# facebook/zstd

Hardware: NVIDIA H100
Metric: compress GB/s (input) at level 1 (higher is better)
Workload: dtype u8

## Files before the change

### zstd_b200/csrc/zb_match.cu

```cuda
#include "zb_device.cuh"
#include "zb_kernels.h"
#include "zb_merge.cuh"

template <bool DICT>
__device__ __forceinline__ u32 zb_count_fwd(const ZbSeg& sg, u32 a, u32 offset, u32 be, u32 lane)
{
    u32 fwd = 0;
    while (true) {
        u32 const pa = a + fwd + 8u * lane;
        u32 m;
        if (pa + 8u <= be) {
            u64 const x = zb_seg_ld64x<DICT>(sg, pa) ^ zb_seg_ld64x<DICT>(sg, pa - offset);
            m = x ? (u32)((__ffsll((long long)x) - 1) >> 3) : 8u;
        } else {
            m = 0;
            while (pa + m < be && zb_seg_byte<DICT>(sg, pa + m) == zb_seg_byte<DICT>(sg, pa + m - offset)) m++;
        }
        u32 const inc = __ballot_sync(ZB_FULL, m != 8u);
        if (inc == 0) { fwd += 256u; continue; }
        int const f = __ffs((int)inc) - 1;
        fwd += 8u * (u32)f + __shfl_sync(ZB_FULL, m, f);
        return fwd;
    }
}
// ... 443 lines not shown
        bool const act = (p < se) && (p + 9u <= be);
        u32 const pp = act ? p : ip;
        u32 dL = act ? zb_dist_at(dLp, fLp, pp - bs) : 0u;
        u32 dS = act ? zb_dist_at(dSp, fSp, pp - bs) : 0u;
        u32 dL1 = act ? zb_dist_at(dLp, fLp, pp + 1u - bs) : 0u;
        if (dL > pp) dL = 0u;
        if (dS > pp) dS = 0u;
        if (dL1 > pp + 1u) dL1 = 0u;
        u64 const w = zb_seg_ld64x<DICT>(sg, pp);
        u32 const cur = (u32)w, cur1 = (u32)(w >> 8);
        bool const v2 = act && rep1 != 0u && (p + 1u >= rep1);
        u32 const r2 = (u32)zb_seg_ld64x<DICT>(sg, v2 ? pp + 1u - rep1 : pp);
        u32 r3 = ~cur;
        bool const v3 = (lane == 0u) && (ip == anchor) && (rep2 != 0u);
        if (ip == anchor && rep2 != 0u) r3 = (u32)zb_seg_ld64x<DICT>(sg, v3 ? pp - rep2 : pp);
        u32 hit = (v3 && r3 == cur) ? 3u : ((v2 && r2 == cur1) ? 2u : (dL ? 1u : (dS ? 4u : 0u)));
        u32 tent = __ballot_sync(ZB_FULL, hit != 0u);
        u32 ms = 0, offset = 0, mlen = 0, wtype = 0;
        bool found = false;
        while (tent) {
            int const winner = __ffs((int)tent) - 1;
            u32 const probe = __shfl_sync(ZB_FULL, p, winner);
            wtype = __shfl_sync(ZB_FULL, hit, winner);
            u32 const wL = __shfl_sync(ZB_FULL, dL, winner), wS = __shfl_sync(ZB_FULL, dS, winner), wL1 = __shfl_sync(ZB_FULL, dL1, winner);
            if (wtype == 3u) { ms = probe; offset = rep2; mlen = 4u + zb_count_fwd<DICT>(sg, probe + 4u, rep2, be, lane); found = true; break; }
            if (wtype == 2u) { ms = probe + 1u; offset = rep1; mlen = 4u + zb_count_fwd<DICT>(sg, probe + 5u, rep1, be, lane); found = true; break; }
            if (wtype == 1u) {
                u32 const f0 = zb_count_fwd<DICT>(sg, probe, wL, be, lane);
                if (f0 >= 8u) {
                    u32 const back = zb_back_coop<DICT>(sg, probe, wL, anchor, lane);
                    ms = probe - back; offset = wL; mlen = back + f0; found = true; break;
                }
                if (lane == (u32)winner) hit = dS ? 4u : 0u;
                if (wS == 0u) { tent &= ~(1u << winner); }
                continue;
            }
            {   u32 const f0 = zb_count_fwd<DICT>(sg, probe, wS, be, lane);
                if (f0 < 4u) { tent &= ~(1u << winner); if (lane == (u32)winner) hit = 0u; continue; }
                u32 mp = probe, mo = wS, ml = f0;
                if (wL1) {
                    u32 const f1 = zb_count_fwd<DICT>(sg, probe + 1u, wL1, be, lane);
                    if (f1 >= 8u && f1 > ml) { mp = probe + 1u; mo = wL1; ml = f1; }
                }
                u32 const back = zb_back_coop<DICT>(sg, mp, mo, anchor, lane);
                ms = mp - back; offset = mo; mlen = back + ml; wtype = 1u; found = true; break;
            }
        }
        if (!found) { ip += 32u * step; continue; }
        if (wtype == 3u) { u32 const t = rep2; rep2 = rep1; rep1 = t; }
        else if (wtype == 1u) { rep2 = rep1; rep1 = offset; }
        if (lane == 0) myseq[nbSeq] = zb_pack_raw(offset, mlen, ms - bs);
        nbSeq++;
        ip = ms + mlen; anchor = ip; searchStart = ip;
    }
    if (lane == 0) { ZbSegMeta z; z.nbSeq = nbSeq; z.pad[0] = z.pad[1] = z.pad[2] = 0; segmeta[(size_t)b * segs + k] = z; }
}

struct ZbRepHist { u32 r1, r2, r3; };
__device__ __forceinline__ u32 zb_rep_code(ZbRepHist& h, u32 off, u32 ll)
{
    u32 code;
    if (ll > 0u) {
        if (off == h.r1) return 1u;
        if (off == h.r2) { code = 2u; h.r2 = h.r1; h.r1 = off; return code; }
        if (off == h.r3) { code = 3u; h.r3 = h.r2; h.r2 = h.r1; h.r1 = off; return code; }
    } else {
        if (off == h.r2) { code = 1u; h.r2 = h.r1; h.r1 = off; return code; }
        if (off == h.r3) { code = 2u; h.r3 = h.r2; h.r2 = h.r1; h.r1 = off; return code; }
        if (h.r1 > 1u && off == h.r1 - 1u) { code = 3u; h.r3 = h.r2; h.r2 = h.r1; h.r1 = off; return code; }
    }
    h.r3 = h.r2; h.r2 = h.r1; h.r1 = off;
    return off + 3u;
}

#ifndef MERGE_MIN_CTAS
#define MERGE_MIN_CTAS 6
#endif
#define SEG_SLOTS (ZB_PARSE_SEG / 4u)

__device__ __forceinline__ u32 zb_block_excl(bool flag, u32* wsum, u32* total)
{
    u32 const lane = threadIdx.x & 31u, warp = threadIdx.x >> 5;
    u32 const bal = __ballot_sync(ZB_FULL, flag);
    if (lane == 0u) wsum[warp] = __popc(bal);
    __syncthreads();
    u32 before = __popc(bal & ((1u << lane) - 1u)), t = 0;
    for (u32 w = 0; w < MERGE_THREADS / 32u; w++) { if (w < warp) before += wsum[w]; t += wsum[w]; }
    __syncthreads();
    *total = t;
    return before;
}

__device__ __forceinline__ void zb_ldm_clip(u32 ms, u32 me, const u64* L, u32 nL, u32* ms2, u32* me2, u32* next, bool* kept)
{
    u32 lo = 0, hi = nL;
    while (lo < hi) { u32 const mid = (lo + hi) >> 1; if (ZB_LDM_START(L[mid]) <= ms) lo = mid + 1u; else hi = mid; }
    bool clipped = false;
    if (lo > 0u && ZB_LDM_START(L[lo - 1u]) + ZB_LDM_LEN(L[lo - 1u]) > ms) { ms = ZB_LDM_START(L[lo - 1u]) + ZB_LDM_LEN(L[lo - 1u]); clipped = true; }
    if (lo < nL && ZB_LDM_START(L[lo]) < me) { me = ZB_LDM_START(L[lo]); clipped = true; }
    *ms2 = ms; *me2 = me; *next = lo;
    *kept = me > ms && (!clipped || me - ms >= 4u);
}
__device__ u32 zb_ldm_overlay(const u64* __restrict__ P, u32 nP, const u64* __restrict__ L, u32 nL, u32* __restrict__ kp, u64* __restrict__ out,
                              u32* wsum, u32* sEnd, u32& carry)
{
    u32 const tid = threadIdx.x;
    u32 base = 0;
    for (u32 i0 = 0; i0 < nP; i0 += MERGE_THREADS) {
        u32 const i = i0 + tid;
        u32 ms2, me2, nx; bool kept = false;
        if (i < nP) { u64 const r = P[i]; zb_ldm_clip(ZB_RAW_MS(r), ZB_RAW_MS(r) + ZB_RAW_MLEN(r), L, nL, &ms2, &me2, &nx, &kept); }
        u32 t;
        u32 const before = zb_block_excl(kept, wsum, &t);
        if (i < nP) kp[i] = base + before;
        base += t;
    }
    if (tid == 0) kp[nP] = base;
    __syncthreads();
    for (u32 i = tid; i < nP; i += MERGE_THREADS) {
        u64 const r = P[i];
        u32 ms2, me2, nx; bool kept;
        zb_ldm_clip(ZB_RAW_MS(r), ZB_RAW_MS(r) + ZB_RAW_MLEN(r), L, nL, &ms2, &me2, &nx, &kept);
        if (kept) out[kp[i] + nx] = zb_pack_ldm(ms2, me2 - ms2, ZB_RAW_OFF(r));
    }
    for (u32 k = tid; k < nL; k += MERGE_THREADS) {
        u32 const s = ZB_LDM_START(L[k]);
        u32 lo = 0, hi = nP;
        while (lo < hi) { u32 const mid = (lo + hi) >> 1; if (ZB_RAW_MS(P[mid]) < s) lo = mid + 1u; else hi = mid; }
        out[k + kp[lo]] = L[k];
    }
    u32 const n = base + nL;
    __syncthreads();
    if (tid == 0) carry = 0;
    for (u32 o0 = 0; o0 < n; o0 += MERGE_THREADS) {
        u32 const o = o0 + tid;
        u64 const m = o < n ? out[o] : 0ull;
        sEnd[tid] = ZB_LDM_START(m) + ZB_LDM_LEN(m);
        __syncthreads();
        u32 const prevEnd = tid ? sEnd[tid - 1u] : carry;
        if (o < n) out[o] = zb_pack_seq(ZB_LDM_OFF(m), ZB_LDM_START(m) - prevEnd, ZB_LDM_LEN(m));
        __syncthreads();
        if (tid == MERGE_THREADS - 1u) carry = sEnd[tid];
        __syncthreads();
    }
    return n;
}

template <bool LDM>
__global__ void __launch_bounds__(MERGE_THREADS, MERGE_MIN_CTAS)
zb_merge_segments_kernel(const u8* __restrict__ src, const ZbDictSlot* __restrict__ dicts, const ZbBlock* __restrict__ blocks, ZbStrides sd, const ZbSegMeta* __restrict__ segmeta,
                         u64* __restrict__ seqs, u8* __restrict__ lits, ZbBlockMeta* __restrict__ meta,
                         ZbLdmView ldm, u32* __restrict__ farScratch, u16* __restrict__ distScratch)
{
    __shared__ u32 sPos[MERGE_TILE], sLit[MERGE_TILE], sLen[MERGE_TILE], sOff[MERGE_TILE];
    __shared__ u32 wsumL[MERGE_THREADS / 32], wsumA[MERGE_THREADS / 32], wmaxU[MERGE_THREADS / 32], wmaxK[MERGE_THREADS / 32];
    __shared__ u32 sR2[MERGE_TILE], sRep[3];
    __shared__ u32 baseL, baseA, carryEnd;
    __shared__ u32 gFirst[ZB_PARSE_SEGS], gCnt[ZB_PARSE_SEGS], gBase[ZB_PARSE_SEGS], gCur[ZB_PARSE_SEGS], gPm[ZB_PARSE_SEGS], gPl[ZB_PARSE_SEGS];
    __shared__ u32 gTotal;
    u32 const b = blockIdx.x, tid = threadIdx.x, lane = tid & 31u, warp = tid >> 5;
    ZbBlock const bd = blocks[b];
    if (bd.size < 7u) return;
    u64* const myseq = seqs + (size_t)b * sd.seq;
    u8*  const mylit = lits + (size_t)b * sd.lit;
    const u8* const in = src + bd.srcOff;
    u32 const segs = (bd.size + ZB_PARSE_SEG - 1u) / ZB_PARSE_SEG;
    u32 const segStride = zb_segsPerRow(sd);
    if (warp == 0u) {
        u32 nb = 0; u64 r0 = 0, rl = 0;
        if (lane < segs) {
            nb = segmeta[(size_t)b * segStride + lane].nbSeq;
            if (nb) { r0 = myseq[(size_t)lane * SEG_SLOTS]; rl = myseq[(size_t)lane * SEG_SLOTS + nb - 1u]; }
        }
        u32 cur = 0, total = 0;
        for (u32 k = 0; k < segs; k++) {
            u32 const n = __shfl_sync(ZB_FULL, nb, (int)k);
            u64 r = __shfl_sync(ZB_FULL, r0, (int)k);
            u64 const last = __shfl_sync(ZB_FULL, rl, (int)k);
            u32 f = 0, pm = 0, pl = 0;
            while (f < n) {
                u32 const ms = ZB_RAW_MS(r), ml = ZB_RAW_MLEN(r);
                if (ms + ml <= cur || (ms < cur && ms + ml - cur < 3u)) { f++; if (f < n) r = myseq[(size_t)k * SEG_SLOTS + f]; continue; }
                if (ms < cur) { pm = cur; pl = ms + ml - cur; } else { pm = ms; pl = ml; }
                break;
            }
            if (lane == 0u) { gFirst[k] = f; gCnt[k] = n - f; gBase[k] = total; gCur[k] = cur; gPm[k] = pm; gPl[k] = pl; }
            if (f < n) { cur = (f == n - 1u) ? pm + pl : ZB_RAW_MS(last) + ZB_RAW_MLEN(last); total += n - f; }
        }
        if (lane == 0u) gTotal = total;
    }
    __syncthreads();
    u32 nbSeq;
    if constexpr (LDM) {
        u64* const P = reinterpret_cast<u64*>(farScratch + (size_t)b * sd.dist);
#pragma unroll 1
        for (u32 k = 0; k < segs; k++) {
            u32 const f = gFirst[k], cnt = gCnt[k];
            const u64* const sfrom = myseq + (size_t)k * SEG_SLOTS + f;
            for (u32 i = tid; i < cnt; i += MERGE_THREADS) {
                u64 r = sfrom[i];
                if (i == 0u) r = zb_pack_raw(ZB_RAW_OFF(r), gPl[k], gPm[k]);
                P[gBase[k] + i] = r;
            }
        }
        __syncthreads();
        nbSeq = zb_ldm_overlay(P, gTotal, ldm.match + ldm.first[b], ldm.cnt[b], reinterpret_cast<u32*>(distScratch + (size_t)b * sd.dist), myseq,
                               wsumA, sPos, carryEnd);
        __syncthreads();
    } else {
#pragma unroll 1
    for (u32 k = 0; k < segs; k++) {
        u32 const f = gFirst[k], cnt = gCnt[k];
        const u64* const sfrom = myseq + (size_t)k * SEG_SLOTS + f;
        u64* const sto = myseq + gBase[k];
        for (u32 c0 = 0; c0 < cnt; c0 += MERGE_THREADS) {
            u32 const i = c0 + tid;
            u64 r = 0; u32 ms = 0, ml = 0;
            if (i < cnt) { r = sfrom[i]; ms = ZB_RAW_MS(r); ml = ZB_RAW_MLEN(r); if (i == 0u) { ms = gPm[k]; ml = gPl[k]; } }
            u32 const myEnd = ms + ml;
            u32 prevEnd = __shfl_up_sync(ZB_FULL, myEnd, 1);
            if (lane == 31u) wsumL[warp] = myEnd;
            __syncthreads();
            if (lane == 0u) prevEnd = warp ? wsumL[warp - 1u] : (c0 ? carryEnd : gCur[k]);
            __syncthreads();
            if (i < cnt) sto[i] = zb_pack_seq(ZB_RAW_OFF(r), ms - prevEnd, ml);
            if (tid == MERGE_THREADS - 1u) carryEnd = myEnd;
            __syncthreads();
        }
    }
    nbSeq = gTotal;
    }
    u32 rep[3] = { 1u, 4u, 8u };
    if (dicts && (bd.flags & ZB_FLAG_FIRST)) { rep[0] = dicts[bd.dictSlot].codeRep[0]; rep[1] = dicts[bd.dictSlot].codeRep[1]; rep[2] = dicts[bd.dictSlot].codeRep[2]; }
    zb_merge_codes(rep[0], rep[1], rep[2], (bd.flags & ZB_FLAG_FIRST) != 0u, myseq, mylit, in, nbSeq, bd.size, meta + b,
                   sPos, sLit, sLen, sOff, sR2, sRep, wsumL, wsumA, wmaxU, wmaxK, baseL, baseA);
}

__global__ void __launch_bounds__(MERGE_THREADS)
zb_merge_small_kernel(const u8* __restrict__ src, const ZbDictSlot* __restrict__ dicts, const ZbBlock* __restrict__ blocks, u32 nbBlocks, ZbStrides sd, const ZbSegMeta* __restrict__ segmeta,
                      u64* __restrict__ seqs, u8* __restrict__ lits, ZbBlockMeta* __restrict__ meta)
{
    u32 const lane = threadIdx.x & 31u;
    u32 const b = blockIdx.x * (MERGE_THREADS / 32u) + (threadIdx.x >> 5);
    if (b >= nbBlocks) return;
    ZbBlock const bd = blocks[b];
    if (bd.size < 7u) return;
    u64* const myseq = seqs + (size_t)b * sd.seq;
    u8* const mylit = lits + (size_t)b * sd.lit;
    const u8* const in = src + bd.srcOff;
    u32 const nbSeq = segmeta[b].nbSeq;
    ZbRepHist hist; hist.r1 = 0; hist.r2 = 0; hist.r3 = 0;
    if (bd.flags & ZB_FLAG_FIRST) {
        hist.r1 = 1u; hist.r2 = 4u; hist.r3 = 8u;
        if (dicts) { hist.r1 = dicts[bd.dictSlot].codeRep[0]; hist.r2 = dicts[bd.dictSlot].codeRep[1]; hist.r3 = dicts[bd.dictSlot].codeRep[2]; }
    }
    u32 posL = 0, posA = 0;
    for (u32 t0 = 0; t0 < nbSeq; t0 += 32u) {
        u32 const i = t0 + lane;
        u64 const r = (i < nbSeq) ? myseq[i] : 0ull;
        u32 const ms = ZB_RAW_MS(r), ml = ZB_RAW_MLEN(r), off = ZB_RAW_OFF(r);
        u32 const myEnd = (i < nbSeq) ? ms + ml : 0u;
        u32 prevEnd = __shfl_up_sync(ZB_FULL, myEnd, 1);
        if (lane == 0u) prevEnd = posA;
        u32 const ll = (i < nbSeq) ? ms - prevEnd : 0u;
        u32 const adv = ll + ((i < nbSeq) ? ml : 0u);
        u32 inL = ll;
#pragma unroll
        for (u32 o = 1; o < 32u; o <<= 1) { u32 const x = __shfl_up_sync(ZB_FULL, inL, o); if (lane >= o) inL += x; }
        u32 code = 0;
        u32 const cnt = min(32u, nbSeq - t0);
        for (u32 j = 0; j < cnt; j++) {
            u32 const o = __shfl_sync(ZB_FULL, off, (int)j), l = __shfl_sync(ZB_FULL, ll, (int)j);
            u32 const c = zb_rep_code(hist, o, l);
            if (lane == j) code = c;
        }
        if (i < nbSeq) {
            const u8* const from = in + prevEnd;
            u8* const to = mylit + posL + inL - ll;
            for (u32 x = 0; x < ll; x++) to[x] = from[x];
            myseq[i] = zb_pack_seq(code, ll, ml);
        }
        posL += __shfl_sync(ZB_FULL, inL, 31);
        posA = __shfl_sync(ZB_FULL, myEnd, (int)(cnt - 1u));
        (void)adv;
    }
    u32 const lastLits = bd.size - posA;
    for (u32 x = lane; x < lastLits; x += 32u) mylit[posL + x] = in[posA + x];
    if (lane == 0) {
        ZbBlockMeta m; m.nbSeq = nbSeq; m.litSize = posL + lastLits; m.litSecSize = 0; m.bodySize = 0;
        m.type = ZB_BT_COMPRESSED; m.forceRaw = 0; m.rleByte = 0; m.pad = 0;
        meta[b] = m;
    }
}

template <int MLS, int P>
static cudaError_t zb_launch_walk_p(const u8* d_src, const ZbDictSlot* d_dicts, const ZbChunk* d_chunks, u32 nbChunks, u32 N, u32 insStep, const ZbStrides& sd,
                                    u32 slotFirstBlock, u16* d_dist, u32* d_far, u32 imageOff, bool build, cudaStream_t stream)
{
    cudaError_t const e = cudaFuncSetAttribute(zb_walk_kernel<MLS, P>, cudaFuncAttributeMaxDynamicSharedMemorySize, 226 * 1024);
    if (e != cudaSuccess) return e;
    zb_walk_kernel<MLS, P><<<nbChunks, ZB_BATCH / P, (size_t)N * 4u, stream>>>(d_src, d_dicts, d_chunks, insStep, N, sd, slotFirstBlock, d_dist, d_far, imageOff, build);
    return cudaGetLastError();
}
template <int MLS>
static cudaError_t zb_launch_walk_m(const u8* d_src, const ZbDictSlot* d_dicts, const ZbChunk* d_chunks, u32 nbChunks, u32 N, u32 insStep, const ZbStrides& sd,
                                    u32 slotFirstBlock, u16* d_dist, u32* d_far, u32 imageOff, bool build, cudaStream_t stream)
{
    size_t const smem = (size_t)N * 4u;
    if (smem <= 56u * 1024u)  return zb_launch_walk_p<MLS, WALK_P_SMALL>(d_src, d_dicts, d_chunks, nbChunks, N, insStep, sd, slotFirstBlock, d_dist, d_far, imageOff, build, stream);
    if (smem <= 113u * 1024u) return zb_launch_walk_p<MLS, WALK_P_MID>(d_src, d_dicts, d_chunks, nbChunks, N, insStep, sd, slotFirstBlock, d_dist, d_far, imageOff, build, stream);
    return zb_launch_walk_p<MLS, 1>(d_src, d_dicts, d_chunks, nbChunks, N, insStep, sd, slotFirstBlock, d_dist, d_far, imageOff, build, stream);
}
extern "C" cudaError_t zb_launch_walk(const u8* d_src, const ZbDictSlot* d_dicts, const ZbChunk* d_chunks, u32 nbChunks, u32 mls, u32 N, u32 insStep, const ZbStrides& sd,
                                      u32 slotFirstBlock, u16* d_dist, u32* d_far, u32 imageOff, bool build, cudaStream_t stream)
{
    switch (mls) {
    case 4: return zb_launch_walk_m<4>(d_src, d_dicts, d_chunks, nbChunks, N, insStep, sd, slotFirstBlock, d_dist, d_far, imageOff, build, stream);
    case 5: return zb_launch_walk_m<5>(d_src, d_dicts, d_chunks, nbChunks, N, insStep, sd, slotFirstBlock, d_dist, d_far, imageOff, build, stream);
    case 6: return zb_launch_walk_m<6>(d_src, d_dicts, d_chunks, nbChunks, N, insStep, sd, slotFirstBlock, d_dist, d_far, imageOff, build, stream);
    case 7: return zb_launch_walk_m<7>(d_src, d_dicts, d_chunks, nbChunks, N, insStep, sd, slotFirstBlock, d_dist, d_far, imageOff, build, stream);
    default: return zb_launch_walk_m<8>(d_src, d_dicts, d_chunks, nbChunks, N, insStep, sd, slotFirstBlock, d_dist, d_far, imageOff, build, stream);
    }
}

extern "C" cudaError_t zb_launch_dict_images(const ZbDictSlot* d_dicts, const ZbChunk* d_imageChunks, u32 nbImages, const ZbParams* prm, cudaStream_t stream)
{
    if (nbImages == 0) return cudaSuccess;
    ZbStrides const sd = zb_strides(ZB_BLOCK_MAX);
    cudaError_t e = zb_launch_walk(nullptr, d_dicts, d_imageChunks, nbImages, prm->mls, prm->tableN, prm->insStep, sd, 0, nullptr, nullptr, 0, true, stream);
    if (e == cudaSuccess && prm->strategy == 2)
        e = zb_launch_walk(nullptr, d_dicts, d_imageChunks, nbImages, 8, prm->tableNLong, prm->insStep, sd, 0, nullptr, nullptr, prm->tableN, true, stream);
    return e;
}

extern "C" cudaError_t zb_launch_match(const u8* d_src, const ZbDictSlot* d_dicts, bool dict, const ZbBlock* d_blocks, u32 nbBlocks,
                                       const ZbChunk* d_chunks, u32 nbChunks, u32 slotFirstBlock, const ZbParams* prm, const ZbWorkRows* rows,
                                       cudaEvent_t evMid, cudaStream_t stream, const ZbLdmView* ldm)
{
    if (nbBlocks == 0) return cudaSuccess;
    ZbStrides const sd = rows->sd;
    u16* const d_dist = rows->dist; u32* const d_far = rows->far; u16* const d_dist2 = rows->dist2; u32* const d_far2 = rows->far2;
    u64* const d_seqs = rows->seqs; ZbBlockMeta* const d_meta = rows->meta; ZbSegMeta* const d_segmeta = rows->segmeta;
    cudaError_t e;
    u32 const segs = zb_segsPerRow(sd);
    u32 const sgrid = (u32)(((u64)nbBlocks * segs + PARSE_WARPS - 1) / PARSE_WARPS);
    if (prm->strategy == 2) {
        e = zb_launch_walk(d_src, d_dicts, d_chunks, nbChunks, 8, prm->tableNLong, prm->insStep, sd, slotFirstBlock, d_dist, d_far, prm->tableN, false, stream); if (e != cudaSuccess) return e;
        e = zb_launch_walk(d_src, d_dicts, d_chunks, nbChunks, prm->mls, prm->tableN, prm->insStep, sd, slotFirstBlock, d_dist2, d_far2, 0, false, stream); if (e != cudaSuccess) return e;
        if (evMid) cudaEventRecord(evMid, stream);
        if (dict) zb_parse_dfast_kernel<true><<<sgrid, 32 * PARSE_WARPS, 0, stream>>>(d_src, d_dicts, d_blocks, nbBlocks, *prm, sd, d_dist, d_far, d_dist2, d_far2, d_seqs, d_meta, d_segmeta);
        else      zb_parse_dfast_kernel<false><<<sgrid, 32 * PARSE_WARPS, 0, stream>>>(d_src, d_dicts, d_blocks, nbBlocks, *prm, sd, d_dist, d_far, d_dist2, d_far2, d_seqs, d_meta, d_segmeta);
    } else {
        if (prm->stepSize < 2u) return cudaErrorInvalidValue;
        e = zb_launch_walk(d_src, d_dicts, d_chunks, nbChunks, prm->mls, prm->tableN, prm->insStep, sd, slotFirstBlock, d_dist, d_far, 0, false, stream); if (e != cudaSuccess) return e;
        if (evMid) cudaEventRecord(evMid, stream);
        if (dict) zb_parse_kernel<true><<<sgrid, 32 * PARSE_WARPS, 0, stream>>>(d_src, d_dicts, d_blocks, nbBlocks, *prm, sd, d_dist, d_far, d_seqs, d_meta, d_segmeta);
        else      zb_parse_kernel<false><<<sgrid, 32 * PARSE_WARPS, 0, stream>>>(d_src, d_dicts, d_blocks, nbBlocks, *prm, sd, d_dist, d_far, d_seqs, d_meta, d_segmeta);
    }
    return zb_launch_merge(d_src, d_dicts, d_blocks, nbBlocks, rows, ldm, stream);
}

extern "C" cudaError_t zb_launch_merge(const u8* d_src, const ZbDictSlot* d_dicts, const ZbBlock* d_blocks, u32 nbBlocks, const ZbWorkRows* rows,
                                       const ZbLdmView* ldm, cudaStream_t stream)
{
    if (nbBlocks == 0) return cudaSuccess;
    ZbStrides const sd = rows->sd;
    u32 const segs = zb_segsPerRow(sd);
    if (segs == 1u && sd.dist <= 8192u)
        zb_merge_small_kernel<<<(nbBlocks + MERGE_THREADS / 32u - 1u) / (MERGE_THREADS / 32u), MERGE_THREADS, 0, stream>>>(d_src, d_dicts, d_blocks, nbBlocks, sd, rows->segmeta, rows->seqs, rows->lits, rows->meta);
    else if (ldm)
        zb_merge_segments_kernel<true><<<nbBlocks, MERGE_THREADS, 0, stream>>>(d_src, d_dicts, d_blocks, sd, rows->segmeta, rows->seqs, rows->lits, rows->meta, *ldm, rows->far, rows->dist);
    else
        zb_merge_segments_kernel<false><<<nbBlocks, MERGE_THREADS, 0, stream>>>(d_src, d_dicts, d_blocks, sd, rows->segmeta, rows->seqs, rows->lits, rows->meta, ZbLdmView(), nullptr, nullptr);
    return cudaGetLastError();
}
```

### zstd_b200/csrc/zb_merge.cuh

```cuda
#ifndef ZB_MERGE_CUH
#define ZB_MERGE_CUH
#include "zb_common.h"
#include "zb_device.cuh"

#define MERGE_THREADS 256
#define MERGE_TILE 1024u
#define MERGE_PER (MERGE_TILE / MERGE_THREADS)

__device__ __forceinline__ void zb_merge_codes(u32 rep0, u32 rep1, u32 rep2, bool first, u64* __restrict__ myseq, u8* __restrict__ mylit,
                                               const u8* __restrict__ in, u32 nbSeq, u32 blockSize, ZbBlockMeta* __restrict__ metaOut,
                                               u32* sPos, u32* sLit, u32* sLen, u32* sOff, u32* sR2, u32* sRep,
                                               u32* wsumL, u32* wsumA, u32* wmaxU, u32* wmaxK, u32& baseL, u32& baseA)
{
    u32 const tid = threadIdx.x, lane = tid & 31u, warp = tid >> 5;
    if (tid == 0) {
        baseL = 0; baseA = 0;
        sRep[0] = first ? rep0 : 0u; sRep[1] = first ? rep1 : 0u; sRep[2] = first ? rep2 : 0u;
    }
    __syncthreads();
    for (u32 t0 = 0; t0 < nbSeq; t0 += MERGE_TILE) {
        u32 const n = min(MERGE_TILE, nbSeq - t0);
        u32 ll[MERGE_PER], adv[MERGE_PER], ml[MERGE_PER], off[MERGE_PER], myL = 0, myA = 0;
#pragma unroll
        for (u32 j = 0; j < MERGE_PER; j++) {
            u32 const i = tid * MERGE_PER + j;
            u64 const q = (i < n) ? myseq[t0 + i] : 0ull;
            ll[j] = ZB_SEQ_LL(q);
            ml[j] = ZB_SEQ_ML(q);
            adv[j] = ll[j] + ml[j];
            off[j] = ZB_SEQ_OFFBASE(q);
            if (i < n) sOff[i] = off[j];
            myL += ll[j]; myA += adv[j];
        }
        u32 inL = myL, inA = myA;
#pragma unroll
        for (u32 o = 1; o < 32u; o <<= 1) {
            u32 const a = __shfl_up_sync(ZB_FULL, inL, o), c = __shfl_up_sync(ZB_FULL, inA, o);
            if (lane >= o) { inL += a; inA += c; }
        }
        if (lane == 31u) { wsumL[warp] = inL; wsumA[warp] = inA; }
        u32 const R1 = sRep[0], R2 = sRep[1], R3 = sRep[2];
        __syncthreads();
        u32 offL = baseL + inL - myL, offA = baseA + inA - myA;
        for (u32 w = 0; w < warp; w++) { offL += wsumL[w]; offA += wsumA[w]; }
#pragma unroll
        for (u32 j = 0; j < MERGE_PER; j++) {
            u32 const i = tid * MERGE_PER + j;
            if (i < n) { sPos[i] = offA; sLit[i] = offL; sLen[i] = ll[j]; }
            offL += ll[j]; offA += adv[j];
        }
        u32 prevOff[MERGE_PER], r2b[MERGE_PER], r3b[MERGE_PER], bef[MERGE_PER];
        bool U[MERGE_PER], K[MERGE_PER];
        u32 run = 0;
#pragma unroll
        for (u32 j = 0; j < MERGE_PER; j++) {
            u32 const i = tid * MERGE_PER + j;
            prevOff[j] = j ? off[j - 1u] : (i == 0u ? R1 : ((i < n) ? sOff[i - 1u] : 0u));
            U[j] = ll[j] > 0u && off[j] == prevOff[j];
            bef[j] = run;
            if (i < n && !U[j]) run = i + 1u;
        }
        {   u32 inc = run;
#pragma unroll
            for (u32 o = 1; o < 32u; o <<= 1) { u32 const x = __shfl_up_sync(ZB_FULL, inc, o); if (lane >= o) inc = max(inc, x); }
            if (lane == 31u) wmaxU[warp] = inc;
            u32 ex = __shfl_up_sync(ZB_FULL, inc, 1); if (lane == 0u) ex = 0u;
            __syncthreads();
            for (u32 w = 0; w < warp; w++) ex = max(ex, wmaxU[w]);
#pragma unroll
            for (u32 j = 0; j < MERGE_PER; j++) {
                u32 const i = tid * MERGE_PER + j;
                u32 const m = max(bef[j], ex);
                r2b[j] = m == 0u ? R2 : (m == 1u ? R1 : sOff[m - 2u]);
                if (i < n) sR2[i] = r2b[j];
            }
        }
        if (tid == MERGE_THREADS - 1u) { baseL = offL; baseA = offA; }
        run = 0;
#pragma unroll
        for (u32 j = 0; j < MERGE_PER; j++) {
            u32 const i = tid * MERGE_PER + j;
            K[j] = U[j] || off[j] == r2b[j];
            bef[j] = run;
            if (i < n && !K[j]) run = i + 1u;
        }
        {   u32 inc = run;
#pragma unroll
            for (u32 o = 1; o < 32u; o <<= 1) { u32 const x = __shfl_up_sync(ZB_FULL, inc, o); if (lane >= o) inc = max(inc, x); }
            if (lane == 31u) wmaxK[warp] = inc;
            u32 ex = __shfl_up_sync(ZB_FULL, inc, 1); if (lane == 0u) ex = 0u;
            __syncthreads();
            for (u32 w = 0; w < warp; w++) ex = max(ex, wmaxK[w]);
#pragma unroll
            for (u32 j = 0; j < MERGE_PER; j++) {
                u32 const i = tid * MERGE_PER + j;
                u32 const m = max(bef[j], ex);
                r3b[j] = m == 0u ? R3 : sR2[m - 1u];
                bool const swp = !U[j] && off[j] == r2b[j];
                u32 c = off[j] + 3u;
                if (ll[j] > 0u) { if (U[j]) c = 1u; else if (swp) c = 2u; else if (off[j] == r3b[j]) c = 3u; }
                else            { if (swp) c = 1u; else if (off[j] == r3b[j]) c = 2u; else if (prevOff[j] > 1u && off[j] == prevOff[j] - 1u) c = 3u; }
                if (i < n) myseq[t0 + i] = zb_pack_seq(c, ll[j], ml[j]);
                if (i == n - 1u) { sRep[0] = off[j]; sRep[1] = U[j] ? r2b[j] : prevOff[j]; sRep[2] = K[j] ? r3b[j] : r2b[j]; }
            }
        }
        {   u32 const L0 = sLit[0], L1 = sLit[n - 1u] + sLen[n - 1u];
            for (u32 g = (L0 >> 3) + tid; (g << 3) < L1; g += MERGE_THREADS) {
                u32 const jb = g << 3;
                u32 const j0 = jb > L0 ? jb : L0, j1 = jb + 8u < L1 ? jb + 8u : L1;
                u32 sq = 0;
#pragma unroll
                for (u32 stp = MERGE_TILE / 2u; stp > 0u; stp >>= 1) {
                    u32 const c = sq + stp;
                    if (c < n && sLit[c] <= j0) sq = c;
                }
                u32 runEnd = sLit[sq] + sLen[sq];
                const u8* from = in + (sPos[sq] - sLit[sq]);
                u64 v = 0;
#pragma unroll
                for (u32 k = 0; k < 8u; k++) {
                    u32 const j = jb + k;
                    if (j >= j0 && j < j1) {
                        while (j >= runEnd) { sq++; runEnd = sLit[sq] + sLen[sq]; from = in + (sPos[sq] - sLit[sq]); }
                        v |= (u64)from[j] << (8u * k);
                    }
                }
                if (j1 - j0 == 8u) *reinterpret_cast<u64*>(mylit + jb) = v;
                else for (u32 j = j0; j < j1; j++) mylit[j] = (u8)(v >> (8u * (j - jb)));
            }
        }
        __syncthreads();
    }
    u32 const litSeq = baseL, consumed = baseA;
    u32 const lastLits = blockSize - consumed;
    for (u32 x = tid; x < lastLits; x += MERGE_THREADS) mylit[litSeq + x] = in[consumed + x];
    if (tid == 0) {
        ZbBlockMeta m; m.nbSeq = nbSeq; m.litSize = litSeq + lastLits; m.litSecSize = 0; m.bodySize = 0;
        m.type = ZB_BT_COMPRESSED; m.forceRaw = 0; m.rleByte = 0; m.pad = 0;
        *metaOut = m;
    }
}
#endif
```

### zstd_b200/csrc/zb_seqimport.cu

```cuda
#include "zb_device.cuh"
#include "zb_kernels.h"
#include "zb_merge.cuh"

#define SEQ_THREADS 256u
#define SEQ_TILE 1024u
#define SEQ_PER (SEQ_TILE / SEQ_THREADS)

__device__ __forceinline__ bool zb_isDelim(uint4 q, bool expl) { return expl && q.x == 0u && q.z == 0u; }

__device__ __forceinline__ void zb_scan2(u64& a, u32& b, u64* wa, u32* wb, u64* totA, u32* totB)
{
    u32 const lane = threadIdx.x & 31u, warp = threadIdx.x >> 5;
#pragma unroll
    for (u32 o = 1; o < 32u; o <<= 1) {
        u64 const x = __shfl_up_sync(ZB_FULL, a, o); u32 const y = __shfl_up_sync(ZB_FULL, b, o);
        if (lane >= o) { a += x; b += y; }
    }
    if (lane == 31u) { wa[warp] = a; wb[warp] = b; }
    __syncthreads();
    u64 pa = 0; u32 pb = 0;
    for (u32 w = 0; w < warp; w++) { pa += wa[w]; pb += wb[w]; }
    if (totA) { u64 ta = 0; u32 tb = 0; for (u32 w = 0; w < blockDim.x / 32u; w++) { ta += wa[w]; tb += wb[w]; } *totA = ta; *totB = tb; }
    a += pa; b += pb;
    __syncthreads();
// ... 12 lines not shown
#pragma unroll
    for (u32 k = 0; k < SEQ_PER; k++) {
        u32 const i = t0 + k * SEQ_THREADS + tid;
        sq[k * SEQ_THREADS + tid] = i < n ? seqs[i] : make_uint4(0u, 0u, 0u, 0u);
    }
    bool prevDelim = false;
    if (tid == 0 && t0 > 0) prevDelim = zb_isDelim(seqs[t0 - 1u], expl);
    __syncthreads();
    u64 len[SEQ_PER]; bool end[SEQ_PER];
    u64 a = 0; u32 c = 0;
#pragma unroll
    for (u32 k = 0; k < SEQ_PER; k++) {
        u32 const j = tid * SEQ_PER + k;
        uint4 const q = sq[j];
        bool const pd = j ? zb_isDelim(sq[j - 1u], expl) : prevDelim;
        bool const d = zb_isDelim(q, expl);
        len[k] = (u64)q.y + q.z;
        end[k] = t0 + j < n && d && (q.y > 0u || (t0 + j > 0u && !pd));
        a += len[k]; c += end[k];
    }
    u64 const myA = a; u32 const myC = c;
    if (!PLACE) {
        u64 ta; u32 tb;
        zb_scan2(a, c, wa, wb, &ta, &tb);
        if (tid == 0) { tileLen[blockIdx.x] = ta; tileEnds[blockIdx.x] = tb; }
        return;
    }
    zb_scan2(a, c, wa, wb, nullptr, nullptr);
    u64 p = tileLen[blockIdx.x] + a - myA;
    u32 k0 = tileEnds[blockIdx.x] + c - myC;
    u32 bad = ~0u;
#pragma unroll
    for (u32 k = 0; k < SEQ_PER; k++) {
        u32 const j = tid * SEQ_PER + k, i = t0 + j;
        if (i >= n) break;
        uint4 const q = sq[j];
        u64 const s = p;
        p += len[k];
        if (!zb_isDelim(q, expl)) {
            u64 const bound = p > window ? window : p + dictContent;
            if (q.x == 0u || q.z < 3u || (u64)q.x > bound || q.x > ZB_SEQ_OFF_MAX) bad = min(bad, i);
        }
        if (p > srcSize) bad = min(bad, i);
        if (expl) {
            if (end[k] && k0 < nbBlocks) { blockEnd[k0] = p; blockSeq[k0] = i; }
            k0 += end[k];
        } else if (p > s && s < srcSize) {
            for (u64 b = (s + blockMax - 1u) / blockMax; b < nbBlocks && b * blockMax < p; b++) { blockFirst[b] = i; blockFirstPos[b] = s; }
        }
    }
    if (bad != ~0u) atomicMin(errIdx, (unsigned long long)bad);
}

__global__ void __launch_bounds__(SEQ_THREADS)
zb_seq_scan_kernel(u64* __restrict__ tileLen, u32* __restrict__ tileEnds, u32 nbTiles, u64* __restrict__ ctrl)
{
    __shared__ u64 wa[SEQ_THREADS / 32u]; __shared__ u32 wb[SEQ_THREADS / 32u];
    __shared__ u64 carryA; __shared__ u32 carryB;
    if (threadIdx.x == 0) { carryA = 0; carryB = 0; }
    __syncthreads();
    for (u32 t0 = 0; t0 < nbTiles; t0 += SEQ_THREADS) {
        u32 const i = t0 + threadIdx.x;
        u64 a = i < nbTiles ? tileLen[i] : 0ull; u32 b = i < nbTiles ? tileEnds[i] : 0u;
        u64 const myA = a; u32 const myB = b;
        u64 ta; u32 tb;
        zb_scan2(a, b, wa, wb, &ta, &tb);
        if (i < nbTiles) { tileLen[i] = carryA + a - myA; tileEnds[i] = carryB + b - myB; }
        __syncthreads();
        if (threadIdx.x == 0) { carryA += ta; carryB += tb; }
        __syncthreads();
    }
    if (threadIdx.x == 0) { ctrl[0] = carryA; ctrl[1] = carryB; }
}

__global__ void zb_seq_blocks_kernel(const u64* __restrict__ blockEnd, const u32* __restrict__ blockSeq, u32 nbBlocks, u32 blockMax, u32 dictFlag,
                                     ZbBlock* __restrict__ blocks, u32* __restrict__ blockFirst, u64* __restrict__ blockFirstPos,
                                     u64* __restrict__ ctrl, unsigned long long* __restrict__ errIdx)
{
    u32 const k = blockIdx.x * blockDim.x + threadIdx.x;
    if (k >= nbBlocks) return;
    u64 const start = k ? blockEnd[k - 1u] : 0ull, e = blockEnd[k];
    if (e - start > blockMax) atomicMin(errIdx, (unsigned long long)blockSeq[k]);
    ZbBlock b; b.srcOff = start; b.size = (u32)min(e - start, (u64)blockMax); b.histLen = 0; b.frame = 0; b.dictLen = 0; b.dictSlot = 0;
    b.flags = (k == 0u ? ZB_FLAG_FIRST | dictFlag : 0u) | (k + 1u == nbBlocks ? ZB_FLAG_LAST : 0u);
    blocks[k] = b;
    blockFirst[k] = k ? blockSeq[k - 1u] + 1u : 0u;
    blockFirstPos[k] = start;
    if (k + 1u == nbBlocks) ctrl[3] = e;
}

__global__ void __launch_bounds__(MERGE_THREADS)
zb_seq_convert_kernel(const u8* __restrict__ src, const ZbBlock* __restrict__ blocks, const u32* __restrict__ blockFirst, const u64* __restrict__ blockFirstPos,
                      const uint4* __restrict__ seqsIn, u32 n, const ZbDictSlot* __restrict__ dicts, ZbStrides sd,
                      u64* __restrict__ seqs, u8* __restrict__ lits, ZbBlockMeta* __restrict__ meta)
{
    __shared__ u32 sPos[MERGE_TILE], sLit[MERGE_TILE], sLen[MERGE_TILE], sOff[MERGE_TILE];
    __shared__ u32 wsumL[MERGE_THREADS / 32], wsumA[MERGE_THREADS / 32], wmaxU[MERGE_THREADS / 32], wmaxK[MERGE_THREADS / 32];
    __shared__ u32 sR2[MERGE_TILE], sRep[3];
    __shared__ u32 baseL, baseA;
    __shared__ u64 wa[MERGE_THREADS / 32]; __shared__ u32 wb[MERGE_THREADS / 32];
    __shared__ long long carryP; __shared__ u32 carryK, carryEnd;
    u32 const b = blockIdx.x, tid = threadIdx.x, lane = tid & 31u, warp = tid >> 5;
    ZbBlock const bd = blocks[b];
    if (bd.size < 7u) {
        if (tid == 0) {
            ZbBlockMeta m; m.nbSeq = 0; m.litSize = bd.size; m.litSecSize = 0; m.bodySize = bd.size;
            m.type = ZB_BT_RAW; m.forceRaw = 1; m.rleByte = 0; m.pad = 0;
            meta[b] = m;
        }
        return;
    }
    u64* const myseq = seqs + (size_t)b * sd.seq;
    u8*  const mylit = lits + (size_t)b * sd.lit;
    const u8* const in = src + bd.srcOff;
    u32 const first = blockFirst[b];
    long long const E = bd.size;
    if (tid == 0) { carryP = first < n ? (long long)blockFirstPos[b] - (long long)bd.srcOff : E; carryK = 0; carryEnd = 0; }
    __syncthreads();
    for (u32 i0 = first; i0 < n; i0 += MERGE_THREADS) {
        u32 const i = i0 + tid;
        uint4 const q = i < n ? seqsIn[i] : make_uint4(0u, 0u, 0u, 0u);
        long long const base = carryP;
        if (base >= E) break;
        u64 a = (u64)q.y + q.z; u32 unused = 0;
        u64 const myLen = a;
        zb_scan2(a, unused, wa, wb, nullptr, nullptr);
        long long const s = base + (long long)(a - myLen), m = s + q.y, e = m + q.z;
        long long const ms = m > 0 ? m : 0, me = e < E ? e : E;
        bool const keep = i < n && s < E && me >= ms + 3;
        u32 const kb = __ballot_sync(ZB_FULL, keep);
        u32 const before = __popc(kb & ((1u << lane) - 1u));
        u32 const kEnd = keep ? (u32)me : 0u;
        u32 inc = kEnd;
#pragma unroll
        for (u32 o = 1; o < 32u; o <<= 1) { u32 const x = __shfl_up_sync(ZB_FULL, inc, o); if (lane >= o) inc = max(inc, x); }
        if (lane == 31u) { wsumL[warp] = __popc(kb); wmaxU[warp] = inc; }
        __syncthreads();
        u32 cnt = carryK, prevEnd = carryEnd;
        for (u32 w = 0; w < warp; w++) { cnt += wsumL[w]; prevEnd = max(prevEnd, wmaxU[w]); }
        u32 ex = __shfl_up_sync(ZB_FULL, inc, 1);
        if (lane > 0u) prevEnd = max(prevEnd, ex);
        if (keep) myseq[cnt + before] = zb_pack_seq(q.x, (u32)ms - prevEnd, (u32)(me - ms));
        __syncthreads();
        if (tid == MERGE_THREADS - 1u) {
            u32 tk = 0, te = carryEnd;
            for (u32 w = 0; w < MERGE_THREADS / 32u; w++) { tk += wsumL[w]; te = max(te, wmaxU[w]); }
            carryK += tk; carryEnd = te; carryP = s + (i < n ? (long long)myLen : 0ll);
            if (i + 1u >= n) carryP = E;
        }
        __syncthreads();
    }
    u32 rep[3] = { 1u, 4u, 8u };
    if (dicts && (bd.flags & ZB_FLAG_FIRST)) { rep[0] = dicts[bd.dictSlot].codeRep[0]; rep[1] = dicts[bd.dictSlot].codeRep[1]; rep[2] = dicts[bd.dictSlot].codeRep[2]; }
    zb_merge_codes(rep[0], rep[1], rep[2], (bd.flags & ZB_FLAG_FIRST) != 0u, myseq, mylit, in, carryK, bd.size, meta + b,
                   sPos, sLit, sLen, sOff, sR2, sRep, wsumL, wsumA, wmaxU, wmaxK, baseL, baseA);
}

extern "C" cudaError_t zb_launch_seq_partition(const void* d_seqs, u32 n, int expl, u64* d_tileLen, u32* d_tileEnds, u64* d_ctrl, cudaStream_t stream)
{
    if (n == 0) return cudaSuccess;
    u32 const nbTiles = (n + SEQ_TILE - 1u) / SEQ_TILE;
    zb_seq_tiles_kernel<false><<<nbTiles, SEQ_THREADS, 0, stream>>>((const uint4*)d_seqs, n, expl != 0, d_tileLen, d_tileEnds, 0, 0, 0, 0, 0,
                                                                   nullptr, nullptr, nullptr, nullptr, nullptr);
    zb_seq_scan_kernel<<<1, SEQ_THREADS, 0, stream>>>(d_tileLen, d_tileEnds, nbTiles, d_ctrl);
    return cudaGetLastError();
}

extern "C" cudaError_t zb_launch_seq_place(const void* d_seqs, u32 n, int expl, const u64* d_tileLen, const u32* d_tileEnds,
                                           u64 srcSize, u64 window, u64 dictContent, u32 blockMax, u32 nbBlocks,
                                           u64* d_blockEnd, u32* d_blockSeq, u32* d_blockFirst, u64* d_blockFirstPos, u64* d_ctrl, cudaStream_t stream)
{
    if (n == 0) return cudaSuccess;
    u32 const nbTiles = (n + SEQ_TILE - 1u) / SEQ_TILE;
    zb_seq_tiles_kernel<true><<<nbTiles, SEQ_THREADS, 0, stream>>>((const uint4*)d_seqs, n, expl != 0, (u64*)d_tileLen, (u32*)d_tileEnds,
                                                                  srcSize, window, dictContent, blockMax, nbBlocks,
                                                                  d_blockEnd, d_blockSeq, d_blockFirst, d_blockFirstPos, (unsigned long long*)(d_ctrl + 2));
    return cudaGetLastError();
}

extern "C" cudaError_t zb_launch_seq_blocks(const u64* d_blockEnd, const u32* d_blockSeq, u32 nbBlocks, u32 blockMax, u32 dictFlag,
                                            ZbBlock* d_blocks, u32* d_blockFirst, u64* d_blockFirstPos, u64* d_ctrl, cudaStream_t stream)
{
    if (nbBlocks == 0) return cudaSuccess;
    zb_seq_blocks_kernel<<<(nbBlocks + 255u) / 256u, 256, 0, stream>>>(d_blockEnd, d_blockSeq, nbBlocks, blockMax, dictFlag, d_blocks, d_blockFirst,
                                                                      d_blockFirstPos, d_ctrl, (unsigned long long*)(d_ctrl + 2));
    return cudaGetLastError();
}

extern "C" cudaError_t zb_launch_seq_convert(const u8* d_src, const ZbBlock* d_blocks, u32 nbBlocks, const u32* d_blockFirst, const u64* d_blockFirstPos,
                                             const void* d_seqs, u32 n, const ZbDictSlot* d_dicts, const ZbWorkRows* rows, cudaStream_t stream)
{
    if (nbBlocks == 0) return cudaSuccess;
    zb_seq_convert_kernel<<<nbBlocks, MERGE_THREADS, 0, stream>>>(d_src, d_blocks, d_blockFirst, d_blockFirstPos, (const uint4*)d_seqs, n, d_dicts, rows->sd,
                                                                 rows->seqs, rows->lits, rows->meta);
    return cudaGetLastError();
}
```

Baseline: 113.9.

## Parallelize segment merge across warps and gather literals with 64-bit loads

Replaces the serial warp-0 scan over parse segments with one warp per segment that finds its first surviving sequence by ballot. A single flat pass then compacts all survivors into the far scratch buffer, using binary search over segment bases and the preceding element for literal length, instead of a per-segment tiled scan with three barriers per tile. The code-merge step reads from that scratch buffer, and literal gathering now copies whole runs with unaligned 64-bit loads rather than byte by byte. This adds scratch traffic on the non-LDM path and relies on an assumption that segment count equals warps per block.

```diff
diff --git a/zstd_b200/csrc/zb_match.cu b/zstd_b200/csrc/zb_match.cu
--- a/zstd_b200/csrc/zb_match.cu
+++ b/zstd_b200/csrc/zb_match.cu
@@ -619,11 +619,13 @@
                          u64* __restrict__ seqs, u8* __restrict__ lits, ZbBlockMeta* __restrict__ meta,
                          ZbLdmView ldm, u32* __restrict__ farScratch, u16* __restrict__ distScratch)
 {
+    static_assert(ZB_PARSE_SEGS == MERGE_THREADS / 32, "step 1 reads one parse segment per warp");
     __shared__ u32 sPos[MERGE_TILE], sLit[MERGE_TILE], sLen[MERGE_TILE], sOff[MERGE_TILE];
     __shared__ u32 wsumL[MERGE_THREADS / 32], wsumA[MERGE_THREADS / 32], wmaxU[MERGE_THREADS / 32], wmaxK[MERGE_THREADS / 32];
     __shared__ u32 sR2[MERGE_TILE], sRep[3];
     __shared__ u32 baseL, baseA, carryEnd;
     __shared__ u32 gFirst[ZB_PARSE_SEGS], gCnt[ZB_PARSE_SEGS], gBase[ZB_PARSE_SEGS], gCur[ZB_PARSE_SEGS], gPm[ZB_PARSE_SEGS], gPl[ZB_PARSE_SEGS];
+    __shared__ u32 gLastMs[ZB_PARSE_SEGS], gLastEnd[ZB_PARSE_SEGS];
     __shared__ u32 gTotal;
     u32 const b = blockIdx.x, tid = threadIdx.x, lane = tid & 31u, warp = tid >> 5;
     ZbBlock const bd = blocks[b];
@@ -632,74 +634,66 @@
     u8*  const mylit = lits + (size_t)b * sd.lit;
     const u8* const in = src + bd.srcOff;
     u32 const segs = (bd.size + ZB_PARSE_SEG - 1u) / ZB_PARSE_SEG;
-    u32 const segStride = zb_segsPerRow(sd);
-    if (warp == 0u) {
-        u32 nb = 0; u64 r0 = 0, rl = 0;
-        if (lane < segs) {
-            nb = segmeta[(size_t)b * segStride + lane].nbSeq;
-            if (nb) { r0 = myseq[(size_t)lane * SEG_SLOTS]; rl = myseq[(size_t)lane * SEG_SLOTS + nb - 1u]; }
-        }
-        u32 cur = 0, total = 0;
-        for (u32 k = 0; k < segs; k++) {
-            u32 const n = __shfl_sync(ZB_FULL, nb, (int)k);
-            u64 r = __shfl_sync(ZB_FULL, r0, (int)k);
-            u64 const last = __shfl_sync(ZB_FULL, rl, (int)k);
-            u32 f = 0, pm = 0, pl = 0;
-            while (f < n) {
-                u32 const ms = ZB_RAW_MS(r), ml = ZB_RAW_MLEN(r);
-                if (ms + ml <= cur || (ms < cur && ms + ml - cur < 3u)) { f++; if (f < n) r = myseq[(size_t)k * SEG_SLOTS + f]; continue; }
-                if (ms < cur) { pm = cur; pl = ms + ml - cur; } else { pm = ms; pl = ml; }
-                break;
-            }
-            if (lane == 0u) { gFirst[k] = f; gCnt[k] = n - f; gBase[k] = total; gCur[k] = cur; gPm[k] = pm; gPl[k] = pl; }
-            if (f < n) { cur = (f == n - 1u) ? pm + pl : ZB_RAW_MS(last) + ZB_RAW_MLEN(last); total += n - f; }
-        }
-        if (lane == 0u) gTotal = total;
-    }
-    __syncthreads();
-    u32 nbSeq;
+    u32 const nb = warp < segs ? segmeta[(size_t)b * zb_segsPerRow(sd) + warp].nbSeq : 0u;
+    const u64* const seg = myseq + (size_t)warp * SEG_SLOTS;
+    u64 r = lane < nb ? seg[lane] : 0ull;
+    if (lane == 0u) {
+        u64 const last = nb ? seg[nb - 1u] : 0ull;
+        gLastMs[warp] = ZB_RAW_MS(last); gLastEnd[warp] = ZB_RAW_MS(last) + ZB_RAW_MLEN(last);
+    }
+    __syncthreads();
+    u32 cur = 0;
+#pragma unroll
+    for (u32 k = 0; k < ZB_PARSE_SEGS - 1u; k++) {
+        u32 const ms = gLastMs[k], e = gLastEnd[k];
+        if (k < warp && !(e <= cur || (ms < cur && e - cur < 3u))) cur = e;
+    }
+    u32 f = 0;
+    for (;;) {
+        u32 const ms = ZB_RAW_MS(r), e = ms + ZB_RAW_MLEN(r);
+        u32 const drop = __ballot_sync(ZB_FULL, f + lane < nb && (e <= cur || (ms < cur && e - cur < 3u)));
+        if (drop != ZB_FULL) { f += __ffs(~drop) - 1u; break; }
+        f += 32u;
+        r = f + lane < nb ? seg[f + lane] : 0ull;
+    }
+    r = __shfl_sync(ZB_FULL, r, (int)(f & 31u));
+    if (lane == 0u) {
+        u32 const ms = ZB_RAW_MS(r), ml = ZB_RAW_MLEN(r);
+        gFirst[warp] = f; gCnt[warp] = nb - f; gCur[warp] = cur;
+        gPm[warp] = ms < cur ? cur : ms; gPl[warp] = ms < cur ? ms + ml - cur : ml;
+    }
+    __syncthreads();
+    if (tid < ZB_PARSE_SEGS) {
+        u32 before = 0, total = 0;
+        for (u32 k = 0; k < ZB_PARSE_SEGS; k++) { before += k < tid ? gCnt[k] : 0u; total += gCnt[k]; }
+        gBase[tid] = before;
+        if (tid == 0u) gTotal = total;
+    }
+    __syncthreads();
+    u64* const P = reinterpret_cast<u64*>(farScratch + (size_t)b * sd.dist);
+    u32 const nbSurv = gTotal;
+    for (u32 i = tid; i < nbSurv; i += MERGE_THREADS) {
+        u32 k = 0;
+#pragma unroll
+        for (u32 st = ZB_PARSE_SEGS / 2u; st > 0u; st >>= 1) if (gBase[k + st] <= i) k += st;
+        u32 const j = i - gBase[k];
+        const u64* const from = myseq + (size_t)k * SEG_SLOTS + gFirst[k] + j;
+        u64 const q = from[0];
+        u64 const qp = (!LDM && j) ? from[-1] : 0ull;
+        u32 ms = ZB_RAW_MS(q), ml = ZB_RAW_MLEN(q), prevEnd = ZB_RAW_MS(qp) + ZB_RAW_MLEN(qp);
+        if (j == 0u) { ms = gPm[k]; ml = gPl[k]; prevEnd = gCur[k]; }
+        P[i] = LDM ? zb_pack_raw(ZB_RAW_OFF(q), ml, ms) : zb_pack_seq(ZB_RAW_OFF(q), ms - prevEnd, ml);
+    }
+    __syncthreads();
+    u32 nbSeq = nbSurv;
     if constexpr (LDM) {
-        u64* const P = reinterpret_cast<u64*>(farScratch + (size_t)b * sd.dist);
-#pragma unroll 1
-        for (u32 k = 0; k < segs; k++) {
-            u32 const f = gFirst[k], cnt = gCnt[k];
-            const u64* const sfrom = myseq + (size_t)k * SEG_SLOTS + f;
-            for (u32 i = tid; i < cnt; i += MERGE_THREADS) {
-                u64 r = sfrom[i];
-                if (i == 0u) r = zb_pack_raw(ZB_RAW_OFF(r), gPl[k], gPm[k]);
-                P[gBase[k] + i] = r;
-            }
-        }
-        __syncthreads();
-        nbSeq = zb_ldm_overlay(P, gTotal, ldm.match + ldm.first[b], ldm.cnt[b], reinterpret_cast<u32*>(distScratch + (size_t)b * sd.dist), myseq,
+        nbSeq = zb_ldm_overlay(P, nbSurv, ldm.match + ldm.first[b], ldm.cnt[b], reinterpret_cast<u32*>(distScratch + (size_t)b * sd.dist), myseq,
                                wsumA, sPos, carryEnd);
         __syncthreads();
-    } else {
-#pragma unroll 1
-    for (u32 k = 0; k < segs; k++) {
-        u32 const f = gFirst[k], cnt = gCnt[k];
-        const u64* const sfrom = myseq + (size_t)k * SEG_SLOTS + f;
-        u64* const sto = myseq + gBase[k];
-        for (u32 c0 = 0; c0 < cnt; c0 += MERGE_THREADS) {
-            u32 const i = c0 + tid;
-            u64 r = 0; u32 ms = 0, ml = 0;
-            if (i < cnt) { r = sfrom[i]; ms = ZB_RAW_MS(r); ml = ZB_RAW_MLEN(r); if (i == 0u) { ms = gPm[k]; ml = gPl[k]; } }
-            u32 const myEnd = ms + ml;
-            u32 prevEnd = __shfl_up_sync(ZB_FULL, myEnd, 1);
-            if (lane == 31u) wsumL[warp] = myEnd;
-            __syncthreads();
-            if (lane == 0u) prevEnd = warp ? wsumL[warp - 1u] : (c0 ? carryEnd : gCur[k]);
-            __syncthreads();
-            if (i < cnt) sto[i] = zb_pack_seq(ZB_RAW_OFF(r), ms - prevEnd, ml);
-            if (tid == MERGE_THREADS - 1u) carryEnd = myEnd;
-            __syncthreads();
-        }
-    }
-    nbSeq = gTotal;
     }
     u32 rep[3] = { 1u, 4u, 8u };
     if (dicts && (bd.flags & ZB_FLAG_FIRST)) { rep[0] = dicts[bd.dictSlot].codeRep[0]; rep[1] = dicts[bd.dictSlot].codeRep[1]; rep[2] = dicts[bd.dictSlot].codeRep[2]; }
-    zb_merge_codes(rep[0], rep[1], rep[2], (bd.flags & ZB_FLAG_FIRST) != 0u, myseq, mylit, in, nbSeq, bd.size, meta + b,
+    zb_merge_codes(rep[0], rep[1], rep[2], (bd.flags & ZB_FLAG_FIRST) != 0u, LDM ? myseq : P, myseq, mylit, in, nbSeq, bd.size, meta + b,
                    sPos, sLit, sLen, sOff, sR2, sRep, wsumL, wsumA, wmaxU, wmaxK, baseL, baseA);
 }
 
@@ -838,6 +832,6 @@
     else if (ldm)
         zb_merge_segments_kernel<true><<<nbBlocks, MERGE_THREADS, 0, stream>>>(d_src, d_dicts, d_blocks, sd, rows->segmeta, rows->seqs, rows->lits, rows->meta, *ldm, rows->far, rows->dist);
     else
-        zb_merge_segments_kernel<false><<<nbBlocks, MERGE_THREADS, 0, stream>>>(d_src, d_dicts, d_blocks, sd, rows->segmeta, rows->seqs, rows->lits, rows->meta, ZbLdmView(), nullptr, nullptr);
+        zb_merge_segments_kernel<false><<<nbBlocks, MERGE_THREADS, 0, stream>>>(d_src, d_dicts, d_blocks, sd, rows->segmeta, rows->seqs, rows->lits, rows->meta, ZbLdmView(), rows->far, nullptr);
     return cudaGetLastError();
 }
diff --git a/zstd_b200/csrc/zb_merge.cuh b/zstd_b200/csrc/zb_merge.cuh
--- a/zstd_b200/csrc/zb_merge.cuh
+++ b/zstd_b200/csrc/zb_merge.cuh
@@ -7,7 +7,7 @@
 #define MERGE_TILE 1024u
 #define MERGE_PER (MERGE_TILE / MERGE_THREADS)
 
-__device__ __forceinline__ void zb_merge_codes(u32 rep0, u32 rep1, u32 rep2, bool first, u64* __restrict__ myseq, u8* __restrict__ mylit,
+__device__ __forceinline__ void zb_merge_codes(u32 rep0, u32 rep1, u32 rep2, bool first, const u64* seqIn, u64* myseq, u8* __restrict__ mylit,
                                                const u8* __restrict__ in, u32 nbSeq, u32 blockSize, ZbBlockMeta* __restrict__ metaOut,
                                                u32* sPos, u32* sLit, u32* sLen, u32* sOff, u32* sR2, u32* sRep,
                                                u32* wsumL, u32* wsumA, u32* wmaxU, u32* wmaxK, u32& baseL, u32& baseA)
@@ -24,7 +24,7 @@
 #pragma unroll
         for (u32 j = 0; j < MERGE_PER; j++) {
             u32 const i = tid * MERGE_PER + j;
-            u64 const q = (i < n) ? myseq[t0 + i] : 0ull;
+            u64 const q = (i < n) ? seqIn[t0 + i] : 0ull;
             ll[j] = ZB_SEQ_LL(q);
             ml[j] = ZB_SEQ_ML(q);
             adv[j] = ll[j] + ml[j];
@@ -117,13 +117,18 @@
                 u32 runEnd = sLit[sq] + sLen[sq];
                 const u8* from = in + (sPos[sq] - sLit[sq]);
                 u64 v = 0;
-#pragma unroll
-                for (u32 k = 0; k < 8u; k++) {
-                    u32 const j = jb + k;
-                    if (j >= j0 && j < j1) {
-                        while (j >= runEnd) { sq++; runEnd = sLit[sq] + sLen[sq]; from = in + (sPos[sq] - sLit[sq]); }
-                        v |= (u64)from[j] << (8u * k);
+                for (u32 j = j0;;) {
+                    u32 const e = runEnd < j1 ? runEnd : j1;
+                    if (e > j) {
+                        u64 w = 0;
+                        if ((u32)(from + j - in) + 8u <= blockSize) w = zb_ld64u(from + j);
+                        else for (u32 x = 0; x < e - j; x++) w |= (u64)from[j + x] << (8u * x);
+                        u32 const nb = e - j;
+                        v |= (nb == 8u ? w : w & ((1ull << (8u * nb)) - 1ull)) << (8u * (j - jb));
+                        j = e;
                     }
+                    if (j >= j1) break;
+                    sq++; runEnd = sLit[sq] + sLen[sq]; from = in + (sPos[sq] - sLit[sq]);
                 }
                 if (j1 - j0 == 8u) *reinterpret_cast<u64*>(mylit + jb) = v;
                 else for (u32 j = j0; j < j1; j++) mylit[j] = (u8)(v >> (8u * (j - jb)));
diff --git a/zstd_b200/csrc/zb_seqimport.cu b/zstd_b200/csrc/zb_seqimport.cu
--- a/zstd_b200/csrc/zb_seqimport.cu
+++ b/zstd_b200/csrc/zb_seqimport.cu
@@ -188,7 +188,7 @@
     }
     u32 rep[3] = { 1u, 4u, 8u };
     if (dicts && (bd.flags & ZB_FLAG_FIRST)) { rep[0] = dicts[bd.dictSlot].codeRep[0]; rep[1] = dicts[bd.dictSlot].codeRep[1]; rep[2] = dicts[bd.dictSlot].codeRep[2]; }
-    zb_merge_codes(rep[0], rep[1], rep[2], (bd.flags & ZB_FLAG_FIRST) != 0u, myseq, mylit, in, carryK, bd.size, meta + b,
+    zb_merge_codes(rep[0], rep[1], rep[2], (bd.flags & ZB_FLAG_FIRST) != 0u, myseq, myseq, mylit, in, carryK, bd.size, meta + b,
                    sPos, sLit, sLen, sOff, sR2, sRep, wsumL, wsumA, wmaxU, wmaxK, baseL, baseA);
 }
 
```

After: 114.5 (median of 6 runs). Within noise of the previous version (+0.6%).
